# saptadeb/botLab

Measured on AMD Instinct MI355X. Metric: SLAM steps/sec (map+MCL+A*), higher is better.
Workload: dtype int8 grid / f32 poses with f64 intermediates / int64 weights; 1 GPU; full SLAM step on 200x200 @5cm grid (continuing from the shipped, already built obstacle_slam_10mx10m_5cm map), 100000 particles, 290 rays, A* replan on; particles=100000, rays=290, pipeline_depth=14, planner_lanes=2, planner_batch=6, parallelism=single GPU, collective=none

## Files before the change

### botlab_amd/_capi.py

```python
import ctypes as C
import os

_HERE = os.path.dirname(os.path.abspath(__file__))
LIB_PATH = os.environ.get("BOTLAB_HIP_LIB") or os.path.join(_HERE, "libbotlab_hip.so")


class Pose(C.Structure):
    _fields_ = [("utime", C.c_int64), ("x", C.c_float), ("y", C.c_float), ("theta", C.c_float)]

    def __repr__(self):
        return f"Pose(utime={self.utime}, x={self.x!r}, y={self.y!r}, theta={self.theta!r})"


class Particle(C.Structure):
    _fields_ = [("pose", Pose), ("parent_pose", Pose), ("weight", C.c_double)]


class Lidar(C.Structure):
    _fields_ = [("utime", C.c_int64), ("num_ranges", C.c_int32), ("ranges", C.POINTER(C.c_float)),
                ("thetas", C.POINTER(C.c_float)), ("times", C.POINTER(C.c_int64)),
                ("intensities", C.POINTER(C.c_float))]


class SearchParams(C.Structure):
# ... 339 lines not shown
    "bl_pf_set_adaptive": (C.c_int, [_vp, _P(PfAdaptiveParams)]),
    "bl_pf_adaptive_state": (C.c_int, [_vp, _P(PfAdaptiveState)]),
    "bl_pf_clusters": (C.c_int, [_vp, _P(PfClusterParams), _P(PfClusters), _vp]),
    "bl_pf_cluster_pose": (C.c_int, [_P(PfCluster), C.c_uint64, _P(PfClusterParams), _P(PfClusterPose)]),
    "bl_pf_set_particles": (C.c_int, [_vp, _vp, _vp]),
    "bl_pf_get_particles": (C.c_int, [_vp, _vp]),
    "bl_pf_set_noise_seed": (C.c_int, [_vp, C.c_uint64]),
    "bl_pf_update": (C.c_int, [_vp, _P(Pose), _P(Lidar), _vp, C.c_int, _vp, _P(Pose)]),
    "bl_pf_update_begin": (C.c_int, [_vp, _P(Pose), _P(Lidar), _vp, C.c_int, _vp, _P(C.c_int)]),
    "bl_pf_update_end": (C.c_int, [_vp, _P(Pose)]),
    "bl_pf_update_action_only": (C.c_int, [_vp, _P(Pose), _vp, _P(Pose)]),
    "bl_pf_pose_estimate": (C.c_int, [_vp, _P(Pose)]),
    "bl_pf_pose_device_ptr": (_vp, [_vp]),
    "bl_pf_estimate_posterior_pose": (C.c_int, [_vp, _vp]),
    "bl_pf_debug_estimate_stats": (C.c_int, [_vp, _vp]),
    "bl_pf_debug_set_finish_generation": (C.c_int, [_vp, C.c_uint32]),
    "bl_pf_set_strict_resampling": (C.c_int, [_vp, C.c_int]),
    "bl_pf_debug_resample": (C.c_int, [_vp, C.c_int, _vp]),
    "bl_pf_debug_enable": (C.c_int, [_vp, C.c_int]),
    "bl_pf_debug_last": (C.c_int, [_vp, _vp, _vp]),
    "bl_pf_debug_uniform_runs": (C.c_int, [_vp, _P(C.c_int)]),
    "bl_debug_trig_addition_probe": (C.c_int, [_vp, C.c_uint64, C.c_uint32, _P(C.c_float), _P(C.c_float), _P(C.c_float), _P(C.c_uint64)]),
    "bl_dist_create": (C.c_int, [_vp, _P(_vp)]),
    "bl_dist_destroy": (None, [_vp]),
    "bl_dist_set_distances": (C.c_int, [_vp, _vp]),
    "bl_dist_download": (C.c_int, [_vp, _vp]),
    "bl_dist_debug_stats": (C.c_int, [_vp, _vp]),
    "bl_dist_forget": (C.c_int, [_vp]),
    "bl_dist_debug_bound": (C.c_int, [_vp, _vp, _vp]),
    "bl_dist_debug_fused": (C.c_int, [_vp, _vp]),
# ... 4 lines not shown
    "bl_dist_metric": (C.c_int, [_vp, _P(C.c_int), _P(C.c_int)]),
    "bl_dist_download_codes": (C.c_int, [_vp, _vp]),
    "bl_dist_table": (C.c_int, [_vp, _vp, _P(C.c_int)]),
    "bl_astar_search": (C.c_int, [_vp, _vp, _P(Pose), _P(Pose), _P(SearchParams), _vp, C.c_int, _P(C.c_int),
                                  _P(C.c_int64)]),
    "bl_astar_set_open_capacity": (C.c_int, [_vp, C.c_int64]),
    "bl_astar_debug_last_kernel": (C.c_int, [_vp]),
    "bl_debug_heap2_replay": (C.c_int, [_vp, _vp, _vp, C.c_int, C.c_int, C.c_int64, _vp, _vp, _P(C.c_int), _vp]),
    "bl_astar_search_async": (C.c_int, [_vp, _vp, _P(Pose), _P(Pose), _P(SearchParams)]),
    "bl_astar_search_async_dev_start": (C.c_int, [_vp, _vp, _vp, _P(Pose), _P(SearchParams)]),
    "bl_astar_search_result": (C.c_int, [_vp, _vp, C.c_int, _P(C.c_int), _P(C.c_int64)]),
    "bl_planner_create": (C.c_int, [_vp, C.c_int, _P(_vp)]),
    "bl_planner_create_batched": (C.c_int, [_vp, C.c_int, C.c_int, _P(_vp)]),
    "bl_planner_destroy": (None, [_vp]),
    "bl_planner_submit": (C.c_int, [_vp, _vp, _vp, _P(Pose), _P(SearchParams)]),
    "bl_planner_fetch": (C.c_int, [_vp, _vp, C.c_int, _P(C.c_int), _P(C.c_int64)]),
    "bl_planner_flush": (C.c_int, [_vp]),
    "bl_planner_timing": (C.c_int, [_vp, C.c_int, _P(C.c_double), _P(C.c_double), _P(C.c_int64)]),
    "bl_planner_submit_with_map_update": (C.c_int, [_vp, _vp, _P(Lidar), _vp, C.c_int64, _vp, _P(Pose), _P(SearchParams)]),
    "bl_mapping_update_finishing_pf": (C.c_int, [_vp, _P(Lidar), _vp, C.c_int64, _vp]),
    "bl_scan_prefetch": (C.c_int, [_vp, _P(Lidar)]),
    "bl_comm_load": (C.c_int, [C.c_char_p]),
    "bl_comm_unique_id": (C.c_int, [C.c_char_p, C.c_char_p]),
    "bl_comm_create": (C.c_int, [_vp, C.c_char_p, C.c_char_p, C.c_int, C.c_int, _P(_vp)]),
    "bl_comm_destroy": (None, [_vp]),
    "bl_comm_all_gather_inplace": (C.c_int, [_vp, _vp, C.c_size_t]),
    "bl_dev_enable_peer_access": (C.c_int, [C.c_int, C.c_int]),
    "bl_dev_alloc": (C.c_int, [_vp, C.c_size_t, _P(_vp)]),
    "bl_dev_word": (C.c_int, [_vp, _vp, C.c_int, _P(C.c_uint32)]),
    "bl_dev_free": (C.c_int, [_vp]),
# ... 217 lines not shown
```

### botlab_amd/csrc/bl_mapping.hip

```cpp
#include <stdio.h>

#include "bl_internal.h"
#include "bl_mcl_finish.h"

#define MAP_THREADS 1024
#define MAP_LDS_COUNTERS (72 * 1024)
#define MAP_MAX_RAYS 8192
#define MAP_CELL_LIMIT (1 << 24)

struct bl_mapping {
    bl_ctx* ctx;
    float max_laser;
    int hit, miss;
    bool initialized;
    int64_t prev_utime;
    bl_pose_xyt_t* d_prev;
    int4* d_rays;
    int ray_capacity;
};

struct map_args {
    int8_t* cells;
    bl_frame frame;
    const float* ranges;
// ... 104 lines not shown
            const int4* s4 = (const int4*)a.cells;
            int4* d4 = (int4*)a.snap_cells;
            for (size_t base = 0; base < n16; base += 4 * MAP_THREADS) {
                int4 v[4];
#pragma unroll
                for (int u = 0; u < 4; ++u) { const size_t i = base + (size_t)u * MAP_THREADS + threadIdx.x; if (i < n16) v[u] = s4[i]; }
#pragma unroll
                for (int u = 0; u < 4; ++u) { const size_t i = base + (size_t)u * MAP_THREADS + threadIdx.x; if (i < n16) d4[i] = v[u]; }
            }
            for (size_t i = n16 * 16 + threadIdx.x; i < n; i += MAP_THREADS) a.snap_cells[i] = a.cells[i];
        }
        if (threadIdx.x == 0) *a.snap_pose = a.fin_on ? s_fin_pose : *a.snap_pose_src;
    }
}

__device__ __forceinline__ int4 map_ray_cells(const map_args& a, const bl_pose3& pb, const bl_pose3& pe, float range, float ray_theta, int64_t ray_time)
{
    int4 ray = make_int4(0x7fffffff, 0, 0, 0);
    if (range <= a.max_laser) {
        bl_pose3 rp = a.interp ? bl_interpolate_pose(pb, pe, bl_interp_ratio(ray_time, a.t_begin, a.t_den)) : pe;
        float theta = bl_wrap_to_pi(rp.theta - ray_theta);
        float sn, cs, sx, sy;
        bl_sincosf(theta, &sn, &cs);
        bl_global_to_grid(rp.x, rp.y, a.frame, &sx, &sy);
        float fx = (range * cs * a.frame.cpm) + sx;
        float fy = (range * sn * a.frame.cpm) + sy;
        const float lim = (float)MAP_CELL_LIMIT;
        if (fx > -lim && fx < lim && fy > -lim && fy < lim && sx > -lim && sx < lim && sy > -lim && sy < lim)
            ray = make_int4((int)sx, (int)sy, (int)fx, (int)fy);
    }
    return ray;
}

__device__ __forceinline__ void map_update_body(const map_args& a, int8_t* snap, const int4 (&sv)[MAP_EARLY_VEC], bl_pose_xyt_t* lds_pose, bool provisional)
{
    extern __shared__ __align__(16) unsigned int s_cnt[];
    __shared__ int s_box[4];
    __shared__ float s_pose[6];
    __shared__ int s_segp[MAP_SEG_RAYS + 1];
    __shared__ int s_wsum[MAP_THREADS / 64];
    __shared__ int s_redo;
    __shared__ int s_dirty[4];

    const int tid = threadIdx.x;
    MSTAMP(0);
    float pre_range = 0.0f, pre_theta = 0.0f;
// ... 15 lines not shown
        s_pose[3] = cur.x; s_pose[4] = cur.y; s_pose[5] = cur.theta;
        s_box[0] = 0x7fffffff; s_box[1] = 0x7fffffff; s_box[2] = -0x7fffffff; s_box[3] = -0x7fffffff;
        s_redo = 0;
        s_dirty[0] = 1; s_dirty[1] = 1; s_dirty[2] = 0; s_dirty[3] = 0;
    }
    __syncthreads();
    if (!a.apply) { if (prov) take_exact_pose(); return 0; }

    const bl_pose3 pb = {s_pose[0], s_pose[1], s_pose[2]};
    const bl_pose3 pe = {s_pose[3], s_pose[4], s_pose[5]};
    const bool seg_walk = a.R <= MAP_SEG_RAYS;

    MSTAMP(1);
    int bx_lo = 0x7fffffff, by_lo = 0x7fffffff, bx_hi = -0x7fffffff, by_hi = -0x7fffffff;
    int4 my_ray = make_int4(0x7fffffff, 0, 0, 0);
    for (int r = tid; r < a.R; r += MAP_THREADS) {
        const bool first = r == tid;
        const int4 ray = map_ray_cells(a, pb, pe, first ? pre_range : a.ranges[r], first ? pre_theta : a.thetas[r],
                                       a.interp ? (first ? pre_time : a.times[r]) : 0);
        if (ray.x != 0x7fffffff) {
            bx_lo = min(bx_lo, min(ray.x, ray.z)); by_lo = min(by_lo, min(ray.y, ray.w));
            bx_hi = max(bx_hi, max(ray.x, ray.z)); by_hi = max(by_hi, max(ray.y, ray.w));
        }
        a.rays[r] = ray;
        my_ray = ray;
    }
    for (int off = 32; off > 0; off >>= 1) {
        bx_lo = min(bx_lo, __shfl_xor(bx_lo, off, 64)); by_lo = min(by_lo, __shfl_xor(by_lo, off, 64));
        bx_hi = max(bx_hi, __shfl_xor(bx_hi, off, 64)); by_hi = max(by_hi, __shfl_xor(by_hi, off, 64));
    }
    if ((tid & 63) == 0 && bx_lo != 0x7fffffff) {
        atomicMin(&s_box[0], bx_lo); atomicMin(&s_box[1], by_lo);
        atomicMax(&s_box[2], bx_hi); atomicMax(&s_box[3], by_hi);
    }
// ... 108 lines not shown
                        const int c = (y - sy0) * ww + (x - bx0);
                        atomicAdd(&s_cnt[c >> 1], (c & 1) ? 0x10000u : 1u);
                    }
                    rem += 2 * dmin;
                    if (rem >= 2 * dmaj) { rem -= 2 * dmaj; n += 1; }
                }
            }
            __syncthreads();
            MSTAMP(5);
            if (prov) {
                XSTAMP(15);
                take_exact_pose();
                XSTAMP(11);
                const bl_pose3 pe2 = {lds_pose->x, lds_pose->y, pe.theta};
                if (tid < a.R) {
                    const int4 ray2 = map_ray_cells(a, pb, pe2, pre_range, pre_theta, pre_time);
                    if (ray2.x != my_ray.x || ray2.y != my_ray.y || ray2.z != my_ray.z || ray2.w != my_ray.w) atomicOr(&s_redo, 1);
                }
                __syncthreads();
                if (s_redo) return 1;
                prov = false;
                XSTAMP(12);
            }
            if (leader) {
                const int M = (int)half_of(s_cnt[ci >> 1], ci);
                int v = a.cells[idx];
                v = max(-128, min(127, v + a.hit * H) - a.miss * M);
                a.cells[idx] = (int8_t)v;
                if (snap) snap[idx] = (int8_t)v;
                if (a.mirror) a.mirror[mirror_at(a, idx, idx_y)] = (int8_t)v;
                atomicAnd(&s_cnt[ci >> 1], (ci & 1) ? 0x0000ffffu : 0xffff0000u);
// ... 315 lines not shown
```

### botlab_amd/csrc/bl_mcl.hip

```cpp
#include <math.h>
#include <stdio.h>
#include <stdlib.h>
#include <string.h>
#include <new>

#include <hip/hip_ext.h>
#define BL_PF_HELPER
#include "bl_internal.h"
#include "bl_mcl_finish.h"

#define MCL_LDS_RAYS 384
#define MCL_BLOCK 512
#define MCL_MIN_BLOCKS 512
#define MCL_ROUND_SHORT_DIV 128
#define MCL_WIN_SMALL_BYTES (64 * 1024)
#define MCL_WIN_MAX 208
#define MCL_WIN_MARGIN 24
#define SCAN_THREADS 256
#define SCAN_ITEMS 2
#define SCAN_TILE (SCAN_THREADS * SCAN_ITEMS)


struct mcl_switches {
    bool no_fused_finish, no_framed, no_mirror_reuse, no_stage_dma, no_stage_x4, no_window, no_fast_trig;
// ... 2571 lines not shown
                ((long long)xs[0] - (long long)gs[0]) * 0.01, ((long long)xs[1] - (long long)st[1]) * 0.01, ((long long)xs[2] - (long long)st[1]) * 0.01);
        fprintf(stderr, "pre-chain wave 0: block sums done %+.2f, past their barrier %+.2f, terms done %+.2f\n", ((long long)xs[8] - (long long)st[0]) * 0.01,
                ((long long)xs[9] - (long long)st[0]) * 0.01, ((long long)xs[10] - (long long)st[0]) * 0.01);
        fprintf(stderr, "pre-chain: sums barrier %+.2f, stepped %+.2f, maps barrier %+.2f after the finisher's entry\n", ((long long)xs[5] - (long long)st[0]) * 0.01,
                ((long long)xs[6] - (long long)st[0]) * 0.01, ((long long)xs[7] - (long long)st[0]) * 0.01);
        fprintf(stderr, "pre-chain published %+.2f, x chain had its start value %+.2f after the finisher's entry\n", ((long long)xs[3] - (long long)st[0]) * 0.01, ((long long)xs[4] - (long long)st[0]) * 0.01);
        fprintf(stderr, "map workgroup: counts stand %+.2f, exact pose taken %+.2f, verified %+.2f, leaders done %+.2f, window done %+.2f after the finisher's entry\n",
                ((long long)xs[15] - (long long)st[0]) * 0.01, ((long long)xs[11] - (long long)st[0]) * 0.01, ((long long)xs[12] - (long long)st[0]) * 0.01,
                ((long long)xs[13] - (long long)st[0]) * 0.01, ((long long)xs[14] - (long long)st[0]) * 0.01);
        fprintf(stderr, "finisher timeline (us): block sums +%.2f, records in and staged +%.2f, lists and gaps +%.2f, chains +%.2f, exit +%.2f\n", (st[1] - st[0]) * 0.01,
                (st[2] - st[1]) * 0.01, (st[3] - st[2]) * 0.01, (st[4] - st[3]) * 0.01, (st[5] - st[4]) * 0.01);
    }
    return BL_OK;
}

extern "C" int bl_pf_debug_set_finish_generation(bl_pf* pf, uint32_t generation)
{
    BL_CHECK_ARG(pf != nullptr);
    pf->fin_gen = generation;
    return BL_OK;
}

extern "C" int bl_pf_set_strict_resampling(bl_pf* pf, int on)
{
    BL_CHECK_ARG(pf != nullptr);
    if (pf->pending_end) { bl_set_error("update pending"); return BL_ERR_STATE; }
    const bool was = pf->strict;
    pf->strict = on != 0;
    if (pf->initialized && was != pf->strict) { BL_HIP(hipSetDevice(pf->ctx->device)); return pf_scan(pf, pf->cur, 0, 0); }
    return BL_OK;
// ... 618 lines not shown
```

### botlab_amd/csrc/bl_mcl_finish.h

```cpp
#ifndef BL_MCL_FINISH_H
#define BL_MCL_FINISH_H

#include "bl_internal.h"
#include "bl_serial_sum.h"

#define UNI_MAX 192
struct uni_seg { double c0, inc, last; int i0, n; };

struct pf_state {
    double S;
    bl_pose_xyt_t pose;
    unsigned int wait_timeouts;
    unsigned int shard_broken;
    double sums_used[5];
    unsigned int chain_stats[8];
    unsigned int lookahead[2];
    unsigned int pre_stats[2];
    unsigned long long cstamps[16];
    unsigned long long gstamps[8];
    unsigned long long stamps[6];
    int uni_n;
    int uni_pad;
    uni_seg uni[UNI_MAX];
    unsigned long long xstamps[16];
// ... 129 lines not shown
    if (mode >= 0) {
        double w = 0.0, last;
        if (mode == 1) w = 1.0 / (double)N;
        else if (S == 2.0 * (double)N) w = w_floor;
        if (w > 0.0) n = uni_build(w, N, st->uni, UNI_MAX, &last);
    }
    st->uni_n = n;
}

#define MCLF_MAXW (MCLF_WG / 64)
struct mclf_smem {
    unsigned long long off[MCLF_MAXW], wave[MCLF_MAXW], tot[MCLF_MAXW];
    double bx[MCLF_MAXW], by[MCLF_MAXW];
    double wx[MCLF_MAXW], wy[MCLF_MAXW];
    double red[MCLF_POSE_THREADS / 64][5];
    float xy[2], first[2];
    unsigned int stats[8];
    int tbase[2][BL_MAX_SHARDS + 1];
    int ntab_seen[2];
    double pre[2][MCLF_PRE_STEPPED * MCLF_SUB];
    double psum[2][MCLF_PRE_SUBS];
    ss_wild pmap[2][MCLF_PRE_SUBS];
};

#ifdef MCLF_STAMPS
#define MCLF_NOW() ((unsigned long long)wall_clock64())
#else
#define MCLF_NOW() 0ull
#endif

__device__ __forceinline__ double mclf_wave_sum(double v)
{
    for (int off = 32; off > 0; off >>= 1) v += __shfl_down(v, off, 64);
    return v;
}
__device__ __forceinline__ double mclf_wave_sum_all(double v)
{
    for (int off = 32; off > 0; off >>= 1) v += __shfl_xor(v, off, 64);
    return v;
}

__device__ __forceinline__ void mclf_store_u64(unsigned long long* p, unsigned long long v)
{
    __hip_atomic_store(p, v, __ATOMIC_RELAXED, __HIP_MEMORY_SCOPE_AGENT);
}
__device__ __forceinline__ unsigned long long mclf_load_u64(const unsigned long long* p)
{
    return __hip_atomic_load(p, __ATOMIC_RELAXED, __HIP_MEMORY_SCOPE_AGENT);
}
__device__ __forceinline__ void mclf_drain_stores()
{
    asm volatile("s_waitcnt vmcnt(0)" ::: "memory");
}
// ... 178 lines not shown
    return v;
}
__device__ __forceinline__ int mclf_wave_min(int v)
{
#define MCLF_STEP(C, R) v = min(v, mclf_dpp<C, R>(0x7fffffff, v));
    MCLF_DPP_STEPS(MCLF_STEP)
#undef MCLF_STEP
    return __builtin_amdgcn_readlane(v, 63);
}
__device__ __forceinline__ int mclf_wave_max(int v)
{
#define MCLF_STEP(C, R) v = max(v, mclf_dpp<C, R>((int)0x80000000, v));
    MCLF_DPP_STEPS(MCLF_STEP)
#undef MCLF_STEP
    return __builtin_amdgcn_readlane(v, 63);
}
__device__ __forceinline__ ss_rec mclf_scan_join(ss_rec r)
{
#define MCLF_STEP(C, R) { const ss_rec o = ss_rec_make(mclf_dpp<C, R>(SS_ID, r.key), mclf_dpp<C, R>(0, r.D), mclf_dpp<C, R>(0, r.lo), mclf_dpp<C, R>(0, r.hi)); \
                          r = ss_rec_join(o, r); }
    MCLF_DPP_STEPS(MCLF_STEP)
#undef MCLF_STEP
    return r;
}
__device__ __forceinline__ ss_rec mclf_scan_join_segmented(ss_rec r, int head)
{
#define MCLF_STEP(C, R) { const ss_rec o = ss_rec_make(mclf_dpp<C, R>(SS_ID, r.key), mclf_dpp<C, R>(0, r.D), mclf_dpp<C, R>(0, r.lo), mclf_dpp<C, R>(0, r.hi)); \
                          const int oh = mclf_dpp<C, R>(0, head);                                                                                      \
                          const ss_rec j = ss_rec_join(o, r);                                                                                          \
                          r.key = head ? r.key : j.key; r.D = head ? r.D : j.D; r.lo = head ? r.lo : j.lo; r.hi = head ? r.hi : j.hi;                  \
// ... 134 lines not shown
        }
#pragma unroll
        for (int q = 0; q < 4; ++q) {
            const int j = j0 + q * gt;
            if (j < f.nblocks) {
                const unsigned long long u = (unsigned long long)pu[q];
                total += u;
                if (j < first_block) { before += u; bx += px4[q]; by += py4[q]; }
            }
        }
    }
#ifdef MCLF_STAMPS
    asm volatile("s_waitcnt vmcnt(0)" ::: "memory");
    if (tid == 0 && g == f.groups / 2) f.state->xstamps[0] = MCLF_NOW();
#endif
    for (int off = 32; off > 0; off >>= 1) { before += __shfl_xor(before, off, 64); total += __shfl_xor(total, off, 64); }
    bx = mclf_wave_sum_all(bx); by = mclf_wave_sum_all(by);
    if (lane == 0) { sm.off[wave] = before; sm.tot[wave] = total; sm.bx[wave] = bx; sm.by[wave] = by; }
    unsigned long long loc[MCLF_ITEMS];
    unsigned long long run = 0;
#pragma unroll
    for (int k = 0; k < MCLF_ITEMS; ++k) { run += __float_as_uint(r[k].w); loc[k] = run; }
    unsigned long long incl = run;
    for (int off = 1; off < 64; off <<= 1) {
        unsigned long long t = __shfl_up(incl, off, 64);
        if (lane >= off) incl += t;
    }
    if (lane == 63) sm.wave[wave] = incl;
    MCLF_GSTAMP(1);
    __syncthreads();
    MCLF_GSTAMP(2);
    unsigned long long off0 = incl - run, S_u = 0;
    double px = 0.0, py = 0.0;
    for (int w = 0; w < nw; ++w) { off0 += sm.off[w]; S_u += sm.tot[w]; px += sm.bx[w]; py += sm.by[w]; if (w < wave) off0 += sm.wave[w]; }
    if (!f.recs) {
#pragma unroll
        for (int k = 0; k < MCLF_ITEMS; ++k)
            if (base + k < hi) f.prefix[base + k] = off0 + loc[k];
        return;
    }
    MCLF_GSTAMP(3);
    const double S = (double)S_u;
    const double St = mclf_term_S(f, S);
    double tx[MCLF_ITEMS], ty[MCLF_ITEMS];
    double sx = 0.0, sy = 0.0;
#pragma unroll
    for (int k = 0; k < MCLF_ITEMS; ++k) {
        tx[k] = mclf_term(r[k], St, 0); ty[k] = mclf_term(r[k], St, 1);
        sx += tx[k]; sy += ty[k];
    }
    sx = mclf_wave_sum_all(sx); sy = mclf_wave_sum_all(sy);
    if (lane == 0) { sm.wx[wave] = sx; sm.wy[wave] = sy; }
    MCLF_GSTAMP(4);
    __syncthreads();
    px /= S; py /= S;
    for (int w = 0; w < wave; ++w) { px += sm.wx[w]; py += sm.wy[w]; }
    const bool very_first = g * nw + wave < MCLF_PRE_SUBS;
    const ss_rec rx = mclf_make_record(f, 0, tx, cnt, px, very_first, lane, g * nw + wave);
    const ss_rec ry = mclf_make_record(f, 1, ty, cnt, py, very_first, lane, g * nw + wave);
    MCLF_GSTAMP(5);
    const bool side_data = (rx.key != SS_ID && (rx.key & MCLF_RISKY) != 0) || (ry.key != SS_ID && (ry.key & MCLF_RISKY) != 0);
    if (side_data) mclf_drain_stores();
    if (lane == 0) {
        const int s = g * nw + wave;
        mclf_store_rec(mclf_rec_ptr(f, 0, s), rx, f.tag);
        mclf_store_rec(mclf_rec_ptr(f, 1, s), ry, f.tag);
// ... 541 lines not shown
                const mclf_tab_elem* row = st->tab + sp.tslot * MCLF_SUB + 2 * lane;
                mclf_tab_elem el[MCLF_ITEMS] = {row[0], row[1]};
                acc = mclf_replay_table(el, sp.tkey, n, 0, acc, lane, &stats[1], &stats[2]);
            } else {
                double t[MCLF_ITEMS];
                mclf_load_terms(f, axis, S, lo, lo + n, lane, t);
                acc = mclf_replay(t, n, 0, sp.tslot <= -2 ? n : 0, acc, lane, &stats[1], lds_terms);
                stats[0] += 1;
            }
        }
        prev = sp.s;
    }
    return acc;
}

__device__ __forceinline__ void mclf_reduce_partials(const mcl_finish_args& f, mclf_smem& sm)
{
    const int tid = threadIdx.x, lane = tid & 63, wave = tid >> 6;
    if (tid < MCLF_POSE_THREADS) {
        double v[5] = {0, 0, 0, 0, 0};
        for (int b0 = tid; b0 < f.nblocks; b0 += 4 * MCLF_POSE_THREADS) {
            double p[4][5];
#pragma unroll
            for (int q = 0; q < 4; ++q) {
                const int b = b0 + q * MCLF_POSE_THREADS;
                const size_t at = (size_t)(b < f.nblocks ? b : 0) * 5;
#pragma unroll
                for (int k = 0; k < 5; ++k) p[q][k] = f.partials[at + k];
            }
#pragma unroll
            for (int q = 0; q < 4; ++q)
                if (b0 + q * MCLF_POSE_THREADS < f.nblocks)
                    for (int k = 0; k < 5; ++k) v[k] += p[q][k];
        }
        for (int k = 0; k < 5; ++k) v[k] = mclf_wave_sum(v[k]);
        if (lane == 0) for (int k = 0; k < 5; ++k) sm.red[wave][k] = v[k];
    }
}
__device__ __forceinline__ void mclf_block_totals(const mclf_smem& sm, double (&tot)[5])
{
    for (int k = 0; k < 5; ++k) tot[k] = 0.0;
    for (int w = 0; w < MCLF_POSE_THREADS / 64; ++w) for (int k = 0; k < 5; ++k) tot[k] += sm.red[w][k];
}
__device__ __forceinline__ bl_pose_xyt_t mclf_approx_pose(const double (&tot)[5], int64_t utime)
{
    bl_pose_xyt_t p;
    p.utime = utime;
    p.x = (float)(tot[1] / tot[0]);
    p.y = (float)(tot[2] / tot[0]);
    p.theta = (float)atan2(tot[3], tot[4]);
    return p;
// ... 62 lines not shown
        for (int k = 0; k < MCLF_ITEMS; ++k) {
            const int i = k < bcnt ? lo + lane * MCLF_ITEMS + k : 0;
            if (!f.sh) { const mclf_f4 v = *(mclf_gptr4)(f.rec + i); br[k] = make_float4(v.x, v.y, v.z, v.w); }
            else br[k] = mclf_particle(f, i);
        }
    }
    if (tid < MCLF_POSE_THREADS) {
        double su = 0.0;
        for (int b0 = tid; b0 < f.nblocks; b0 += 4 * MCLF_POSE_THREADS) {
            double p[4];
#pragma unroll
            for (int q = 0; q < 4; ++q) { const int b = b0 + q * MCLF_POSE_THREADS; p[q] = f.partials[(size_t)(b < f.nblocks ? b : 0) * 5]; }
#pragma unroll
            for (int q = 0; q < 4; ++q) if (b0 + q * MCLF_POSE_THREADS < f.nblocks) su += p[q];
        }
        su = mclf_wave_sum_all(su);
        if (lane == 0) sm.red[wave][0] = su;
    }
#ifdef MCLF_STAMPS
    if (tid == 0) f.state->xstamps[8] = MCLF_NOW();
#endif
    __syncthreads();
#ifdef MCLF_STAMPS
    if (tid == 0) f.state->xstamps[9] = MCLF_NOW();
#endif
    double S = 0.0;
    for (int w = 0; w < MCLF_POSE_THREADS / 64; ++w) S += sm.red[w][0];
    S = mclf_term_S(f, S);
    double bt[MCLF_ITEMS] = {0.0, 0.0};
    double* pre = sm.pre[axis];
    int nstep = 0;
    if (stepper) {
#pragma unroll
        for (int q = 0; q < MCLF_PRE_STEPPED; ++q) {
            double qs = 0.0;
            if (q < npre) {
#pragma unroll
                for (int k = 0; k < MCLF_ITEMS; ++k) {
                    const double t = (lane * MCLF_ITEMS + k < cnt[q]) ? mclf_term(pre_r[q][k], S, axis) : 0.0;
                    pre[q * MCLF_SUB + 2 * lane + k] = t;
                    qs += t;
                }
                nstep = q * MCLF_SUB + cnt[q];
            }
            qs = mclf_wave_sum_all(qs);
            if (lane == 0) sm.psum[axis][q] = qs;
        }
    } else if (builder) {
        double qs = 0.0;
#pragma unroll
        for (int k = 0; k < MCLF_ITEMS; ++k) { bt[k] = k < bcnt ? mclf_term(br[k], S, axis) : 0.0; qs += bt[k]; }
        qs = mclf_wave_sum_all(qs);
        if (lane == 0) sm.psum[axis][bq] = qs;
    }
#ifdef MCLF_STAMPS
    if (tid == 0) f.state->xstamps[10] = MCLF_NOW();
#endif
    __syncthreads();
#ifdef MCLF_STAMPS
    if (tid == 0) f.state->xstamps[5] = MCLF_NOW();
#endif
    unsigned int ph = 0;
    float v = 0.0f;
    if (stepper) {
        nstep = __builtin_amdgcn_readfirstlane(nstep);
        int i = 0;
        for (; i + 8 <= nstep; i += 8) {
// ... 51 lines not shown
#endif
    }
}

__device__ __forceinline__ void mclf_pose(const mcl_finish_args& f, mclf_smem& sm, char* scratch, size_t scratch_bytes,
                                          bool publish = false)
{
    const int tid = threadIdx.x, lane = tid & 63, wave = tid >> 6;
#ifdef MCLF_STAMPS
    unsigned long long stamp[6] = {MCLF_NOW(), 0, 0, 0, 0, 0};
#define MCLF_STAMP(i) stamp[i] = MCLF_NOW()
#else
#define MCLF_STAMP(i) do { } while (0)
#endif
    const int nrec = f.groups * (f.gthreads >> 6), nbatch = (nrec + 63) >> 6;
    mclf_reduce_partials(f, sm);
    const size_t per_axis = (mclf_stage_bytes(nbatch) + 15) & ~(size_t)15;
    const bool staged = scratch != nullptr && 2 * per_axis <= scratch_bytes;
#define MCLF_STAGE(axis) mclf_stage_at(scratch + (size_t)(axis) * per_axis, nbatch)
    if (staged && tid < 2) *MCLF_STAGE(tid).nent = 0;
    if (tid == 0) {
        const int world = mclf_world(f);
        for (int axis = 0; axis < 2; ++axis) {
            int run = 0;
            for (int r = 0; r < world; ++r) { sm.tbase[axis][r] = run; run += f.sh ? mclf_tab_count(f, 0ull, r, axis) : MCLF_TSLOTS; }
            sm.tbase[axis][world] = run;
            sm.ntab_seen[axis] = 0;
        }
    }
    __syncthreads();
    double S = 0.0;
    for (int w = 0; w < MCLF_POSE_THREADS / 64; ++w) S += sm.red[w][0];
    S = mclf_term_S(f, S);
    MCLF_STAMP(1);
    const int sh_world = mclf_world(f);
    {
        const bool poll = f.groups_wait > 0;
        const int nb2 = 2 * nbatch;
        const void* const dummy = (const void*)mclf_rec_ptr(f, 0, 0);
        for (int round = 0; round * 4 * MCLF_MAXW < nb2; ++round) {
            const void* pr[4];
            bool mine[4];
#pragma unroll
            for (int u = 0; u < 4; ++u) {
                const int it = wave + (4 * round + u) * MCLF_MAXW;
                pr[u] = dummy; mine[u] = false;
                if (it < nb2) {
                    const int axis = it >= nbatch ? 1 : 0, b = it - axis * nbatch;
                    if (b * 64 + lane < nrec) { pr[u] = (const void*)mclf_rec_ptr(f, axis, b * 64 + lane); mine[u] = true; }
// ... 136 lines not shown
    }
    if (wave < 2) {
        unsigned int stats[4] = {0, 0, 0, 0};
        unsigned long long fw;
        unsigned int spins = 0;
        while ((((fw = mclf_load_u64(f.sync + 1 + wave)) >> 32) & 1ull) == 0ull) {
            if (++spins > MCLF_SPIN_LIMIT) { if (lane == 0) atomicAdd(&f.state->wait_timeouts, 1u); break; }
            __builtin_amdgcn_s_sleep(1);
        }
#ifdef MCLF_STAMPS
        if (tid == 0) f.state->xstamps[4] = MCLF_NOW();
#endif
        const float first = __uint_as_float((unsigned int)fw);
        const mclf_stage mine = MCLF_STAGE(wave);
        const float v = mclf_chain(f, staged ? &mine : nullptr, wave ? ntab[1] : ntab[0], wave, S, first, lane, stats, trees[wave], &sm.pre[wave][0]);
        if (lane == 0) { sm.xy[wave] = v; for (int k = 0; k < 4; ++k) sm.stats[4 * wave + k] = stats[k]; }
    }
    __syncthreads();
    MCLF_STAMP(4);
    if (tid == 0) {
        mclf_store_u64(f.sync, 0ull);
        mclf_store_u64(f.sync + 1, 0ull);
        mclf_store_u64(f.sync + 2, 0ull);
        double tot[5] = {0, 0, 0, 0, 0};
        for (int w = 0; w < MCLF_POSE_THREADS / 64; ++w) for (int k = 0; k < 5; ++k) tot[k] += sm.red[w][k];
        f.state->S = tot[0];
        bl_pose_xyt_t p;
        p.utime = f.utime;
        p.x = sm.xy[0];
        p.y = sm.xy[1];
        p.theta = (float)atan2(tot[3], tot[4]);
        f.state->pose = p;
        if (publish) {
            mclf_store_u64(f.sync + 3, (unsigned long long)__float_as_uint(p.x) | (1ull << 32));
            mclf_store_u64(f.sync + 4, (unsigned long long)__float_as_uint(p.y) | (1ull << 32));
        }
        for (int k = 0; k < 5; ++k) f.state->sums_used[k] = tot[k];
        for (int k = 0; k < 8; ++k) f.state->chain_stats[k] = sm.stats[k];
        uni_update(f.state, f.N, tot[0], f.uni_mode, f.w_floor);
#ifdef MCLF_STAMPS
        stamp[5] = MCLF_NOW();
        for (int k = 0; k < 6; ++k) f.state->stamps[k] = stamp[k];
#endif
    }
}
#endif

int bl_pf_take_finish(bl_pf* pf, mcl_finish_args* out);
bl_ctx* bl_pf_ctx(bl_pf* pf);
int bl_pf_launch_taken_finish(bl_pf* pf, const mcl_finish_args* fin);
void bl_pf_ride_launched(bl_pf* pf);
// ... 3 lines not shown
```

### botlab_amd/csrc/bl_planning.hip

```cpp
#include <math.h>
#include <stdio.h>
#include <stdlib.h>
#include <string.h>
#include <cmath>
#include <deque>
#include <map>

#include "bl_internal.h"

struct bl_dist {
    bl_ctx* ctx;
    bl_frame frame;
    size_t capacity;
    uint16_t* row;
    uint16_t* l1;
    float* cells;
    bool floats_valid;
    bool floats_handed_out;
    float* lut;
    int32_t* closed;
    uint32_t closed_gen;
    int* sum_f; int* sum_b; size_t sum_cap;
    int lut_n;
    std::vector<float>* lut_host;
// ... 2786 lines not shown
    bool slot_used[PLANNER_SLOTS];
    int64_t batches;
    int filled;
};

struct planner_ticket { int lane, unit; };

struct bl_planner {
    bl_ctx* main;
    int lanes, batch;
    planner_lane lane[PLANNER_MAX_LANES];
    int cur_lane;
    int64_t submitted, fetched;
    std::deque<planner_ticket>* tickets;
    bool reserved;
};

extern "C" int bl_planner_create_batched(bl_ctx* ctx, int lanes, int batch, bl_planner** out)
{
    BL_CHECK_ARG(ctx != nullptr && out != nullptr && lanes >= 1 && lanes <= PLANNER_MAX_LANES);
    BL_CHECK_ARG(batch >= 1 && batch <= PLANNER_MAX_BATCH);
    BL_HIP(hipSetDevice(ctx->device));
    bl_planner* p = new bl_planner();
    memset((void*)p, 0, sizeof(*p));
    p->main = ctx;
    p->lanes = lanes;
    p->batch = batch;
    p->tickets = new std::deque<planner_ticket>();
    for (int l = 0; l < lanes; ++l) {
        planner_lane& L = p->lane[l];
// ... 111 lines not shown
        BL_HIP(hipStreamSynchronize(L.side->stream));
        bl_grid_destroy(snap);
        snap = nullptr;
    }
    if (!snap) {
        int rc = bl_grid_create(U.ctx, map->frame.width, map->frame.height, map->frame.mpc, map->frame.cpm, map->frame.ox,
                                map->frame.oy, &snap);
        if (rc) return rc;
        BL_HIP(hipStreamSynchronize(L.side->stream));
    }
    snap->frame = map->frame;
    if (L.slot_used[slot] && hipEventQuery(L.slot_free[slot]) != hipSuccess)
        BL_HIP(hipStreamWaitEvent(p->main->stream, L.slot_free[slot], 0));
    out->grid = snap;
    out->cells = snap->cells;
    snap->mirror_valid = false;
    out->pose = U.pose[slot];
    p->reserved = true;
    return BL_OK;
}

void bl_planner_cancel(bl_planner* p) { if (p) p->reserved = false; }

int bl_planner_commit(bl_planner* p, const bl_pose_xyt_t* goal, const bl_search_params_t* params)
{
    BL_CHECK_ARG(p != nullptr && goal != nullptr && params != nullptr);
    if (!p->reserved) { bl_set_error("bl_planner_commit without bl_planner_reserve"); return BL_ERR_STATE; }
    p->reserved = false;
    const int l = p->cur_lane;
    planner_lane& L = p->lane[l];
    planner_unit& U = L.unit[L.filled];
    const int slot = (int)(L.batches % PLANNER_SLOTS);
    const bool deferred = p->batch > 1;
    if (!deferred) {
        BL_HIP(hipEventRecord(U.snap_ready[slot], p->main->stream));
        BL_HIP(hipStreamWaitEvent(L.side->stream, U.snap_ready[slot], 0));
        const int rc = bl_dist_set_distances(U.dist, U.snap[slot]);
// ... 314 lines not shown
```

### botlab_amd/host.py

```python
import ctypes as C
import math

import numpy as np

from . import _capi
from ._capi import Lidar, Particle, Pose, SearchParams, check

_libc = C.CDLL(None)
_libc.rand.restype = C.c_int

PARTICLE_DTYPE = np.dtype([("utime", "<i8"), ("x", "<f4"), ("y", "<f4"), ("theta", "<f4"), ("_pad0", "<f4"),
                           ("p_utime", "<i8"), ("p_x", "<f4"), ("p_y", "<f4"), ("p_theta", "<f4"), ("_pad1", "<f4"),
                           ("weight", "<f8")])
POSE_DTYPE = np.dtype([("utime", "<i8"), ("x", "<f4"), ("y", "<f4"), ("theta", "<f4"), ("_pad", "<f4")])
assert PARTICLE_DTYPE.itemsize == 56 and POSE_DTYPE.itemsize == 24


def make_pose(x=0.0, y=0.0, theta=0.0, utime=0):
    return Pose(int(utime), float(np.float32(x)), float(np.float32(y)), float(np.float32(theta)))


class LidarScan:

    def __init__(self, ranges, thetas, times, utime=0):
# ... 354 lines not shown

    def debugResample(self, rand_value):
        idx = np.empty(self._counts()[1] if self._adaptive_used else self.N, np.int32)
        check(self.ctx.lib.bl_pf_debug_resample(self.h, int(rand_value), idx.ctypes.data))
        return idx

    def debugUniformRuns(self):
        n = C.c_int()
        check(self.ctx.lib.bl_pf_debug_uniform_runs(self.h, C.byref(n)))
        return n.value

    def debugEstimateStats(self):
        out = np.zeros(8, np.uint32)
        check(self.ctx.lib.bl_pf_debug_estimate_stats(self.h, out.ctypes.data))
        return [int(v) for v in out]

    def particles(self):
        out = np.zeros(self._counts()[0], dtype=PARTICLE_DTYPE)
        check(self.ctx.lib.bl_pf_get_particles(self.h, out.ctypes.data))
        return out

    def debugEnable(self, on=True):
        check(self.ctx.lib.bl_pf_debug_enable(self.h, 1 if on else 0))

    def debugLast(self):
        n = self._counts()[0]
        idx = np.empty(n, np.int32)
        like = np.empty(n, np.int32)
        check(self.ctx.lib.bl_pf_debug_last(self.h, idx.ctypes.data, like.ctypes.data))
        return idx, like
# ... 1333 lines not shown
        check(self.ctx.lib.bl_planner_submit_with_map_update(self.h, mapping.h, C.byref(c), pose_dev, int(pose_utime), grid.h,
                                                             C.byref(goal), C.byref(self.searchParams_)))

    def submit_with_map_update_finishing(self, mapping, scan, pf, pose_utime, grid, goal):
        c = scan.as_c()
        check(self.ctx.lib.bl_planner_submit_with_map_update_finishing_pf(self.h, mapping.h, C.byref(c), pf.h, int(pose_utime),
                                                                          grid.h, C.byref(goal), C.byref(self.searchParams_)))

    def fetch(self, return_stats=False):
        n = C.c_int()
        stats = (C.c_int64 * 2)()
        check(self.ctx.lib.bl_planner_fetch(self.h, self._buf, 4097, C.byref(n), stats))
        path = [Pose(p.utime, p.x, p.y, p.theta) for p in self._buf[:min(n.value, 4097)]]
        return (path, (stats[0], stats[1])) if return_stats else path

    def flush(self):
        check(self.ctx.lib.bl_planner_flush(self.h))

    def timing(self, on=-1):
        d, a, n = C.c_double(), C.c_double(), C.c_int64()
        check(self.ctx.lib.bl_planner_timing(self.h, on, C.byref(d), C.byref(a), C.byref(n)))
        return d.value, a.value, n.value

    def close(self):
        if self.h:
            self.ctx.lib.bl_planner_destroy(self.h)
            self.h = None


class MotionPlannerParams:
# ... 197 lines not shown
```

### include/botlab_hip.h

```cpp
#ifndef BOTLAB_HIP_H
#define BOTLAB_HIP_H

#include <math.h>
#include <stddef.h>
#include <stdint.h>

#ifdef __cplusplus
extern "C" {
#endif

#define BL_OK 0
#define BL_ERR_HIP 1
#define BL_ERR_ARG 2
#define BL_ERR_CAPACITY 3
#define BL_ERR_STATE 4

const char* bl_last_error(void);
const char* bl_version(void);

typedef struct bl_pose_xyt_t {
    int64_t utime;
    float x, y, theta;
} bl_pose_xyt_t;

// ... 158 lines not shown
}
int bl_pf_set_particles(bl_pf* pf, const bl_particle_t* particles, const uint32_t* units);
int bl_pf_get_particles(bl_pf* pf, bl_particle_t* out_local);
int bl_pf_set_noise_seed(bl_pf* pf, uint64_t seed);

int bl_pf_update(bl_pf* pf, const bl_pose_xyt_t* odometry, const bl_lidar_t* scan, const bl_grid* map, int rand_value,
                 const float* noise, bl_pose_xyt_t* out_pose);
int bl_pf_update_begin(bl_pf* pf, const bl_pose_xyt_t* odometry, const bl_lidar_t* scan, const bl_grid* map,
                       int rand_value, const float* noise, int* moved);
int bl_pf_update_end(bl_pf* pf, bl_pose_xyt_t* out_pose);
int bl_pf_update_action_only(bl_pf* pf, const bl_pose_xyt_t* odometry, const float* noise, bl_pose_xyt_t* out_pose);
int bl_pf_pose_estimate(bl_pf* pf, bl_pose_xyt_t* out_pose);
const void* bl_pf_pose_device_ptr(bl_pf* pf);
int bl_pf_estimate_posterior_pose(bl_pf* pf, bl_pose_xyt_t* out_pose);
int bl_pf_debug_estimate_stats(bl_pf* pf, uint32_t* out8);
int bl_pf_debug_set_finish_generation(bl_pf* pf, uint32_t generation);
int bl_pf_debug_uniform_runs(bl_pf* pf, int* out_runs);
int bl_pf_set_strict_resampling(bl_pf* pf, int on);
int bl_pf_debug_resample(bl_pf* pf, int rand_value, int32_t* out_idx);
int bl_pf_debug_enable(bl_pf* pf, int on);
int bl_debug_trig_addition_probe(bl_ctx* ctx, uint64_t pairs, uint32_t seed, float* max_sin_err, float* max_cos_err, float* eps_used,
                                 uint64_t* pairs_checked);
int bl_pf_debug_last(bl_pf* pf, int32_t* resample_idx, int32_t* likelihood_half_units);

typedef struct bl_scan_match_params_t {
    int32_t nx, ny;
    int32_t ntheta;
    float   dtheta;
    float   max_range;
    int32_t min_score;
// ... 131 lines not shown
int bl_debug_heap2_replay(bl_ctx* ctx, const int32_t* keys, const uint32_t* pays, int n, int cfg, int64_t capacity,
                          uint32_t* out_keys, uint32_t* out_pays, int* out_n, uint64_t* cycles);
int bl_astar_search_async(bl_ctx* ctx, const bl_dist* distances, const bl_pose_xyt_t* start, const bl_pose_xyt_t* goal,
                          const bl_search_params_t* params);
int bl_astar_search_async_dev_start(bl_ctx* ctx, const bl_dist* distances, const void* d_start ,
                                    const bl_pose_xyt_t* goal, const bl_search_params_t* params);
int bl_astar_search_result(bl_ctx* ctx, bl_pose_xyt_t* out_path, int cap, int* out_len, int64_t* stats);

typedef struct bl_planner bl_planner;
int bl_planner_create(bl_ctx* ctx, int lanes, bl_planner** out);
int bl_planner_create_batched(bl_ctx* ctx, int lanes, int batch, bl_planner** out);
void bl_planner_destroy(bl_planner* p);
int bl_planner_submit(bl_planner* p, const bl_grid* map, const void* d_start_pose ,
                      const bl_pose_xyt_t* goal, const bl_search_params_t* params);
int bl_planner_fetch(bl_planner* p, bl_pose_xyt_t* out_path, int cap, int* out_len, int64_t* stats);
int bl_planner_flush(bl_planner* p);
int bl_planner_timing(bl_planner* p, int on, double* dist_ms, double* astar_ms, int64_t* launches);
int bl_planner_submit_with_map_update(bl_planner* p, bl_mapping* m, const bl_lidar_t* scan, const void* d_pose,
                                      int64_t pose_utime, bl_grid* map, const bl_pose_xyt_t* goal,
                                      const bl_search_params_t* params);
typedef struct bl_comm bl_comm;
int bl_comm_load(const char* rccl_path);
int bl_comm_unique_id(const char* rccl_path, char* out_id128);
int bl_comm_create(bl_ctx* ctx, const char* rccl_path, const char* id128, int rank, int world, bl_comm** out);
void bl_comm_destroy(bl_comm* c);
int bl_comm_all_gather_inplace(bl_comm* c, void* rec, size_t per_rank_floats);

int bl_dev_enable_peer_access(int device, int peer_device);
int bl_dev_alloc(bl_ctx* ctx, size_t bytes, void** out);
int bl_dev_free(void* dev_ptr);
// ... 490 lines not shown
```

Baseline: 12390 steps/s.

## Publish MCL pose per-axis early, DPP wave reductions, reuse ray trig in mapping redo

The MCL finish kernel now publishes each pose axis to the sync slots as soon as its chain finishes, instead of after the final pose assembly. This lets waiting mapping or planning work start sooner. Wave-wide shuffle reductions and scans are replaced with DPP-based u64/f64 scans. The partials reduction is split so that only the normalizer is summed before the barrier and the remaining four sums are reduced later. Mapping caches each ray's trig extent so the provisional-pose redo check only redoes the translation. Debug accessors for lookahead state and the planner snapshot are also added.

```diff
diff --git a/botlab_amd/_capi.py b/botlab_amd/_capi.py
--- a/botlab_amd/_capi.py
+++ b/botlab_amd/_capi.py
@@ -377,6 +377,7 @@
     "bl_pf_pose_device_ptr": (_vp, [_vp]),
     "bl_pf_estimate_posterior_pose": (C.c_int, [_vp, _vp]),
     "bl_pf_debug_estimate_stats": (C.c_int, [_vp, _vp]),
+    "bl_pf_debug_lookahead": (C.c_int, [_vp, _vp]),
     "bl_pf_debug_set_finish_generation": (C.c_int, [_vp, C.c_uint32]),
     "bl_pf_set_strict_resampling": (C.c_int, [_vp, C.c_int]),
     "bl_pf_debug_resample": (C.c_int, [_vp, C.c_int, _vp]),
@@ -411,6 +412,7 @@
     "bl_planner_create_batched": (C.c_int, [_vp, C.c_int, C.c_int, _P(_vp)]),
     "bl_planner_destroy": (None, [_vp]),
     "bl_planner_submit": (C.c_int, [_vp, _vp, _vp, _P(Pose), _P(SearchParams)]),
+    "bl_planner_debug_snapshot": (C.c_int, [_vp, _vp, C.c_int64]),
     "bl_planner_fetch": (C.c_int, [_vp, _vp, C.c_int, _P(C.c_int), _P(C.c_int64)]),
     "bl_planner_flush": (C.c_int, [_vp]),
     "bl_planner_timing": (C.c_int, [_vp, C.c_int, _P(C.c_double), _P(C.c_double), _P(C.c_int64)]),
diff --git a/botlab_amd/csrc/bl_mapping.hip b/botlab_amd/csrc/bl_mapping.hip
--- a/botlab_amd/csrc/bl_mapping.hip
+++ b/botlab_amd/csrc/bl_mapping.hip
@@ -142,22 +142,39 @@
     }
 }
 
-__device__ __forceinline__ int4 map_ray_cells(const map_args& a, const bl_pose3& pb, const bl_pose3& pe, float range, float ray_theta, int64_t ray_time)
+struct map_ray_reach { float ex, ey; double ratio; bool on; };
+__device__ __forceinline__ map_ray_reach map_ray_angle(const map_args& a, const bl_pose3& pb, const bl_pose3& pe, float range, float ray_theta, int64_t ray_time)
+{
+    map_ray_reach d = {0.0f, 0.0f, 0.0, range <= a.max_laser};
+    if (d.on) {
+        if (a.interp) d.ratio = bl_interp_ratio(ray_time, a.t_begin, a.t_den);
+        const float rp_theta = a.interp ? bl_interpolate_pose(pb, pe, d.ratio).theta : pe.theta;
+        float theta = bl_wrap_to_pi(rp_theta - ray_theta);
+        float sn, cs;
+        bl_sincosf(theta, &sn, &cs);
+        d.ex = range * cs * a.frame.cpm;
+        d.ey = range * sn * a.frame.cpm;
+    }
+    return d;
+}
+__device__ __forceinline__ int4 map_ray_place(const map_args& a, const bl_pose3& pb, const bl_pose3& pe, const map_ray_reach& d)
 {
     int4 ray = make_int4(0x7fffffff, 0, 0, 0);
-    if (range <= a.max_laser) {
-        bl_pose3 rp = a.interp ? bl_interpolate_pose(pb, pe, bl_interp_ratio(ray_time, a.t_begin, a.t_den)) : pe;
-        float theta = bl_wrap_to_pi(rp.theta - ray_theta);
-        float sn, cs, sx, sy;
-        bl_sincosf(theta, &sn, &cs);
+    if (d.on) {
+        const bl_pose3 rp = a.interp ? bl_interpolate_pose(pb, pe, d.ratio) : pe;
+        float sx, sy;
         bl_global_to_grid(rp.x, rp.y, a.frame, &sx, &sy);
-        float fx = (range * cs * a.frame.cpm) + sx;
-        float fy = (range * sn * a.frame.cpm) + sy;
+        float fx = d.ex + sx;
+        float fy = d.ey + sy;
         const float lim = (float)MAP_CELL_LIMIT;
         if (fx > -lim && fx < lim && fy > -lim && fy < lim && sx > -lim && sx < lim && sy > -lim && sy < lim)
             ray = make_int4((int)sx, (int)sy, (int)fx, (int)fy);
     }
     return ray;
+}
+__device__ __forceinline__ int4 map_ray_cells(const map_args& a, const bl_pose3& pb, const bl_pose3& pe, float range, float ray_theta, int64_t ray_time)
+{
+    return map_ray_place(a, pb, pe, map_ray_angle(a, pb, pe, range, ray_theta, ray_time));
 }
 
 __device__ __forceinline__ void map_update_body(const map_args& a, int8_t* snap, const int4 (&sv)[MAP_EARLY_VEC], bl_pose_xyt_t* lds_pose, bool provisional)
@@ -203,10 +220,13 @@
     MSTAMP(1);
     int bx_lo = 0x7fffffff, by_lo = 0x7fffffff, bx_hi = -0x7fffffff, by_hi = -0x7fffffff;
     int4 my_ray = make_int4(0x7fffffff, 0, 0, 0);
+    map_ray_reach my_reach = {0.0f, 0.0f, 0.0, false};
     for (int r = tid; r < a.R; r += MAP_THREADS) {
         const bool first = r == tid;
-        const int4 ray = map_ray_cells(a, pb, pe, first ? pre_range : a.ranges[r], first ? pre_theta : a.thetas[r],
-                                       a.interp ? (first ? pre_time : a.times[r]) : 0);
+        const map_ray_reach reach = map_ray_angle(a, pb, pe, first ? pre_range : a.ranges[r], first ? pre_theta : a.thetas[r],
+                                                  a.interp ? (first ? pre_time : a.times[r]) : 0);
+        if (first) my_reach = reach;
+        const int4 ray = map_ray_place(a, pb, pe, reach);
         if (ray.x != 0x7fffffff) {
             bx_lo = min(bx_lo, min(ray.x, ray.z)); by_lo = min(by_lo, min(ray.y, ray.w));
             bx_hi = max(bx_hi, max(ray.x, ray.z)); by_hi = max(by_hi, max(ray.y, ray.w));
@@ -345,7 +365,7 @@
                 XSTAMP(11);
                 const bl_pose3 pe2 = {lds_pose->x, lds_pose->y, pe.theta};
                 if (tid < a.R) {
-                    const int4 ray2 = map_ray_cells(a, pb, pe2, pre_range, pre_theta, pre_time);
+                    const int4 ray2 = map_ray_place(a, pb, pe2, my_reach);
                     if (ray2.x != my_ray.x || ray2.y != my_ray.y || ray2.z != my_ray.z || ray2.w != my_ray.w) atomicOr(&s_redo, 1);
                 }
                 __syncthreads();
diff --git a/botlab_amd/csrc/bl_mcl.hip b/botlab_amd/csrc/bl_mcl.hip
--- a/botlab_amd/csrc/bl_mcl.hip
+++ b/botlab_amd/csrc/bl_mcl.hip
@@ -2609,6 +2609,15 @@
     return BL_OK;
 }
 
+extern "C" int bl_pf_debug_lookahead(bl_pf* pf, uint32_t* out2)
+{
+    BL_CHECK_ARG(pf != nullptr && out2 != nullptr && pf->state != nullptr);
+    BL_HIP(hipSetDevice(pf->ctx->device));
+    BL_HIP(hipStreamSynchronize(pf->ctx->stream));
+    BL_HIP(hipMemcpy(out2, pf->state->lookahead, 2 * sizeof(uint32_t), hipMemcpyDeviceToHost));
+    return BL_OK;
+}
+
 extern "C" int bl_pf_debug_set_finish_generation(bl_pf* pf, uint32_t generation)
 {
     BL_CHECK_ARG(pf != nullptr);
diff --git a/botlab_amd/csrc/bl_mcl_finish.h b/botlab_amd/csrc/bl_mcl_finish.h
--- a/botlab_amd/csrc/bl_mcl_finish.h
+++ b/botlab_amd/csrc/bl_mcl_finish.h
@@ -167,6 +167,7 @@
     double bx[MCLF_MAXW], by[MCLF_MAXW];
     double wx[MCLF_MAXW], wy[MCLF_MAXW];
     double red[MCLF_POSE_THREADS / 64][5];
+    double sred[MCLF_POSE_THREADS / 64];
     float xy[2], first[2];
     unsigned int stats[8];
     int tbase[2][BL_MAX_SHARDS + 1];
@@ -185,11 +186,6 @@
 __device__ __forceinline__ double mclf_wave_sum(double v)
 {
     for (int off = 32; off > 0; off >>= 1) v += __shfl_down(v, off, 64);
-    return v;
-}
-__device__ __forceinline__ double mclf_wave_sum_all(double v)
-{
-    for (int off = 32; off > 0; off >>= 1) v += __shfl_xor(v, off, 64);
     return v;
 }
 
@@ -398,6 +394,34 @@
     MCLF_DPP_STEPS(MCLF_STEP)
 #undef MCLF_STEP
     return __builtin_amdgcn_readlane(v, 63);
+}
+template <int CTRL, int ROW_MASK>
+__device__ __forceinline__ unsigned long long mclf_dpp_u64(unsigned long long v)
+{
+    const int lo = mclf_dpp<CTRL, ROW_MASK>(0, (int)(unsigned int)v), hi = mclf_dpp<CTRL, ROW_MASK>(0, (int)(unsigned int)(v >> 32));
+    return ((unsigned long long)(unsigned int)hi << 32) | (unsigned long long)(unsigned int)lo;
+}
+__device__ __forceinline__ unsigned long long mclf_scan_add_u64(unsigned long long v)
+{
+#define MCLF_STEP(C, R) v += mclf_dpp_u64<C, R>(v);
+    MCLF_DPP_STEPS(MCLF_STEP)
+#undef MCLF_STEP
+    return v;
+}
+__device__ __forceinline__ unsigned long long mclf_wave_sum_u64(unsigned long long v)
+{
+    return (unsigned long long)mclf_readlane_i64_((long long)mclf_scan_add_u64(v), 63);
+}
+__device__ __forceinline__ double mclf_scan_add_f64(double v)
+{
+#define MCLF_STEP(C, R) v += __longlong_as_double((long long)mclf_dpp_u64<C, R>((unsigned long long)__double_as_longlong(v)));
+    MCLF_DPP_STEPS(MCLF_STEP)
+#undef MCLF_STEP
+    return v;
+}
+__device__ __forceinline__ double mclf_wave_sum_f64(double v)
+{
+    return __longlong_as_double(mclf_readlane_i64_(__double_as_longlong(mclf_scan_add_f64(v)), 63));
 }
 __device__ __forceinline__ ss_rec mclf_scan_join(ss_rec r)
 {
@@ -562,18 +586,14 @@
     asm volatile("s_waitcnt vmcnt(0)" ::: "memory");
     if (tid == 0 && g == f.groups / 2) f.state->xstamps[0] = MCLF_NOW();
 #endif
-    for (int off = 32; off > 0; off >>= 1) { before += __shfl_xor(before, off, 64); total += __shfl_xor(total, off, 64); }
-    bx = mclf_wave_sum_all(bx); by = mclf_wave_sum_all(by);
+    before = mclf_wave_sum_u64(before); total = mclf_wave_sum_u64(total);
+    bx = mclf_wave_sum_f64(bx); by = mclf_wave_sum_f64(by);
     if (lane == 0) { sm.off[wave] = before; sm.tot[wave] = total; sm.bx[wave] = bx; sm.by[wave] = by; }
     unsigned long long loc[MCLF_ITEMS];
     unsigned long long run = 0;
 #pragma unroll
     for (int k = 0; k < MCLF_ITEMS; ++k) { run += __float_as_uint(r[k].w); loc[k] = run; }
-    unsigned long long incl = run;
-    for (int off = 1; off < 64; off <<= 1) {
-        unsigned long long t = __shfl_up(incl, off, 64);
-        if (lane >= off) incl += t;
-    }
+    const unsigned long long incl = mclf_scan_add_u64(run);
     if (lane == 63) sm.wave[wave] = incl;
     MCLF_GSTAMP(1);
     __syncthreads();
@@ -597,7 +617,7 @@
         tx[k] = mclf_term(r[k], St, 0); ty[k] = mclf_term(r[k], St, 1);
         sx += tx[k]; sy += ty[k];
     }
-    sx = mclf_wave_sum_all(sx); sy = mclf_wave_sum_all(sy);
+    sx = mclf_wave_sum_f64(sx); sy = mclf_wave_sum_f64(sy);
     if (lane == 0) { sm.wx[wave] = sx; sm.wy[wave] = sy; }
     MCLF_GSTAMP(4);
     __syncthreads();
@@ -1169,27 +1189,36 @@
     return acc;
 }
 
+__device__ __forceinline__ void mclf_partials_thread(const mcl_finish_args& f, int vt, double (&v)[5])
+{
+    for (int k = 0; k < 5; ++k) v[k] = 0.0;
+    for (int b0 = vt; b0 < f.nblocks; b0 += 4 * MCLF_POSE_THREADS) {
+        double p[4][5];
+#pragma unroll
+        for (int q = 0; q < 4; ++q) {
+            const int b = b0 + q * MCLF_POSE_THREADS;
+            const size_t at = (size_t)(b < f.nblocks ? b : 0) * 5;
+#pragma unroll
+            for (int k = 0; k < 5; ++k) p[q][k] = f.partials[at + k];
+        }
+#pragma unroll
+        for (int q = 0; q < 4; ++q)
+            if (b0 + q * MCLF_POSE_THREADS < f.nblocks)
+                for (int k = 0; k < 5; ++k) v[k] += p[q][k];
+    }
+}
+__device__ __forceinline__ void mclf_partials_waves(mclf_smem& sm, double (&v)[5], int vwave, int lane)
+{
+    for (int k = 0; k < 5; ++k) v[k] = mclf_wave_sum(v[k]);
+    if (lane == 0) for (int k = 0; k < 5; ++k) sm.red[vwave][k] = v[k];
+}
 __device__ __forceinline__ void mclf_reduce_partials(const mcl_finish_args& f, mclf_smem& sm)
 {
     const int tid = threadIdx.x, lane = tid & 63, wave = tid >> 6;
     if (tid < MCLF_POSE_THREADS) {
-        double v[5] = {0, 0, 0, 0, 0};
-        for (int b0 = tid; b0 < f.nblocks; b0 += 4 * MCLF_POSE_THREADS) {
-            double p[4][5];
-#pragma unroll
-            for (int q = 0; q < 4; ++q) {
-                const int b = b0 + q * MCLF_POSE_THREADS;
-                const size_t at = (size_t)(b < f.nblocks ? b : 0) * 5;
-#pragma unroll
-                for (int k = 0; k < 5; ++k) p[q][k] = f.partials[at + k];
-            }
-#pragma unroll
-            for (int q = 0; q < 4; ++q)
-                if (b0 + q * MCLF_POSE_THREADS < f.nblocks)
-                    for (int k = 0; k < 5; ++k) v[k] += p[q][k];
-        }
-        for (int k = 0; k < 5; ++k) v[k] = mclf_wave_sum(v[k]);
-        if (lane == 0) for (int k = 0; k < 5; ++k) sm.red[wave][k] = v[k];
+        double v[5];
+        mclf_partials_thread(f, tid, v);
+        mclf_partials_waves(sm, v, wave, lane);
     }
 }
 __device__ __forceinline__ void mclf_block_totals(const mclf_smem& sm, double (&tot)[5])
@@ -1282,7 +1311,7 @@
 #pragma unroll
             for (int q = 0; q < 4; ++q) if (b0 + q * MCLF_POSE_THREADS < f.nblocks) su += p[q];
         }
-        su = mclf_wave_sum_all(su);
+        su = mclf_wave_sum_f64(su);
         if (lane == 0) sm.red[wave][0] = su;
     }
 #ifdef MCLF_STAMPS
@@ -1311,14 +1340,14 @@
                 }
                 nstep = q * MCLF_SUB + cnt[q];
             }
-            qs = mclf_wave_sum_all(qs);
+            qs = mclf_wave_sum_f64(qs);
             if (lane == 0) sm.psum[axis][q] = qs;
         }
     } else if (builder) {
         double qs = 0.0;
 #pragma unroll
         for (int k = 0; k < MCLF_ITEMS; ++k) { bt[k] = k < bcnt ? mclf_term(br[k], S, axis) : 0.0; qs += bt[k]; }
-        qs = mclf_wave_sum_all(qs);
+        qs = mclf_wave_sum_f64(qs);
         if (lane == 0) sm.psum[axis][bq] = qs;
     }
 #ifdef MCLF_STAMPS
@@ -1400,7 +1429,13 @@
 #define MCLF_STAMP(i) do { } while (0)
 #endif
     const int nrec = f.groups * (f.gthreads >> 6), nbatch = (nrec + 63) >> 6;
-    mclf_reduce_partials(f, sm);
+    const int pt = tid - (MCLF_WG - MCLF_POSE_THREADS);
+    double pv[5] = {0, 0, 0, 0, 0};
+    if (pt >= 0) {
+        mclf_partials_thread(f, pt, pv);
+        const double su = mclf_wave_sum_f64(pv[0]);
+        if (lane == 0) sm.sred[pt >> 6] = su;
+    }
     const size_t per_axis = (mclf_stage_bytes(nbatch) + 15) & ~(size_t)15;
     const bool staged = scratch != nullptr && 2 * per_axis <= scratch_bytes;
 #define MCLF_STAGE(axis) mclf_stage_at(scratch + (size_t)(axis) * per_axis, nbatch)
@@ -1416,9 +1451,10 @@
     }
     __syncthreads();
     double S = 0.0;
-    for (int w = 0; w < MCLF_POSE_THREADS / 64; ++w) S += sm.red[w][0];
+    for (int w = 0; w < MCLF_POSE_THREADS / 64; ++w) S += sm.sred[w];
     S = mclf_term_S(f, S);
     MCLF_STAMP(1);
+    if (pt >= 0) mclf_partials_waves(sm, pv, pt >> 6, lane);
     const int sh_world = mclf_world(f);
     {
         const bool poll = f.groups_wait > 0;
@@ -1585,7 +1621,11 @@
         const float first = __uint_as_float((unsigned int)fw);
         const mclf_stage mine = MCLF_STAGE(wave);
         const float v = mclf_chain(f, staged ? &mine : nullptr, wave ? ntab[1] : ntab[0], wave, S, first, lane, stats, trees[wave], &sm.pre[wave][0]);
-        if (lane == 0) { sm.xy[wave] = v; for (int k = 0; k < 4; ++k) sm.stats[4 * wave + k] = stats[k]; }
+        if (lane == 0) {
+            if (publish) mclf_store_u64(f.sync + 3 + wave, (unsigned long long)__float_as_uint(v) | (1ull << 32));
+            sm.xy[wave] = v;
+            for (int k = 0; k < 4; ++k) sm.stats[4 * wave + k] = stats[k];
+        }
     }
     __syncthreads();
     MCLF_STAMP(4);
@@ -1602,10 +1642,6 @@
         p.y = sm.xy[1];
         p.theta = (float)atan2(tot[3], tot[4]);
         f.state->pose = p;
-        if (publish) {
-            mclf_store_u64(f.sync + 3, (unsigned long long)__float_as_uint(p.x) | (1ull << 32));
-            mclf_store_u64(f.sync + 4, (unsigned long long)__float_as_uint(p.y) | (1ull << 32));
-        }
         for (int k = 0; k < 5; ++k) f.state->sums_used[k] = tot[k];
         for (int k = 0; k < 8; ++k) f.state->chain_stats[k] = sm.stats[k];
         uni_update(f.state, f.N, tot[0], f.uni_mode, f.w_floor);
diff --git a/botlab_amd/csrc/bl_planning.hip b/botlab_amd/csrc/bl_planning.hip
--- a/botlab_amd/csrc/bl_planning.hip
+++ b/botlab_amd/csrc/bl_planning.hip
@@ -2824,6 +2824,7 @@
     int64_t submitted, fetched;
     std::deque<planner_ticket>* tickets;
     bool reserved;
+    bl_grid* last_snap;
 };
 
 extern "C" int bl_planner_create_batched(bl_ctx* ctx, int lanes, int batch, bl_planner** out)
@@ -2965,6 +2966,7 @@
         BL_HIP(hipStreamWaitEvent(p->main->stream, L.slot_free[slot], 0));
     out->grid = snap;
     out->cells = snap->cells;
+    p->last_snap = snap;
     snap->mirror_valid = false;
     out->pose = U.pose[slot];
     p->reserved = true;
@@ -2972,6 +2974,18 @@
 }
 
 void bl_planner_cancel(bl_planner* p) { if (p) p->reserved = false; }
+
+extern "C" int bl_planner_debug_snapshot(bl_planner* p, int8_t* out_cells, int64_t n_cells)
+{
+    BL_CHECK_ARG(p != nullptr && out_cells != nullptr);
+    if (!p->last_snap) { bl_set_error("bl_planner_debug_snapshot: nothing has been submitted"); return BL_ERR_STATE; }
+    const bl_frame& f = p->last_snap->frame;
+    BL_CHECK_ARG(n_cells == (int64_t)f.width * f.height);
+    BL_HIP(hipSetDevice(p->main->device));
+    BL_HIP(hipStreamSynchronize(p->main->stream));
+    BL_HIP(hipMemcpy(out_cells, p->last_snap->cells, (size_t)n_cells, hipMemcpyDeviceToHost));
+    return BL_OK;
+}
 
 int bl_planner_commit(bl_planner* p, const bl_pose_xyt_t* goal, const bl_search_params_t* params)
 {
diff --git a/botlab_amd/host.py b/botlab_amd/host.py
--- a/botlab_amd/host.py
+++ b/botlab_amd/host.py
@@ -392,6 +392,11 @@
         out = np.zeros(8, np.uint32)
         check(self.ctx.lib.bl_pf_debug_estimate_stats(self.h, out.ctypes.data))
         return [int(v) for v in out]
+
+    def debugLookahead(self):
+        out = np.zeros(2, np.uint32)
+        check(self.ctx.lib.bl_pf_debug_lookahead(self.h, out.ctypes.data))
+        return int(out[0]), int(out[1])
 
     def particles(self):
         out = np.zeros(self._counts()[0], dtype=PARTICLE_DTYPE)
@@ -1755,6 +1760,11 @@
         path = [Pose(p.utime, p.x, p.y, p.theta) for p in self._buf[:min(n.value, 4097)]]
         return (path, (stats[0], stats[1])) if return_stats else path
 
+    def debugSnapshot(self, grid):
+        out = np.zeros((grid.height, grid.width), np.int8)
+        check(self.ctx.lib.bl_planner_debug_snapshot(self.h, out.ctypes.data, out.size))
+        return out
+
     def flush(self):
         check(self.ctx.lib.bl_planner_flush(self.h))
 
diff --git a/include/botlab_hip.h b/include/botlab_hip.h
--- a/include/botlab_hip.h
+++ b/include/botlab_hip.h
@@ -196,6 +196,7 @@
 const void* bl_pf_pose_device_ptr(bl_pf* pf);
 int bl_pf_estimate_posterior_pose(bl_pf* pf, bl_pose_xyt_t* out_pose);
 int bl_pf_debug_estimate_stats(bl_pf* pf, uint32_t* out8);
+int bl_pf_debug_lookahead(bl_pf* pf, uint32_t out[2]);
 int bl_pf_debug_set_finish_generation(bl_pf* pf, uint32_t generation);
 int bl_pf_debug_uniform_runs(bl_pf* pf, int* out_runs);
 int bl_pf_set_strict_resampling(bl_pf* pf, int on);
@@ -357,6 +358,7 @@
 int bl_planner_submit(bl_planner* p, const bl_grid* map, const void* d_start_pose ,
                       const bl_pose_xyt_t* goal, const bl_search_params_t* params);
 int bl_planner_fetch(bl_planner* p, bl_pose_xyt_t* out_path, int cap, int* out_len, int64_t* stats);
+int bl_planner_debug_snapshot(bl_planner* p, int8_t* out_cells, int64_t n_cells);
 int bl_planner_flush(bl_planner* p);
 int bl_planner_timing(bl_planner* p, int on, double* dist_ms, double* astar_ms, int64_t* launches);
 int bl_planner_submit_with_map_update(bl_planner* p, bl_mapping* m, const bl_lidar_t* scan, const void* d_pose,
```

After: 12590 steps/s, median of 6. 1.7% higher.
